# YiyanXu/DiFashion

Hardware: AMD Instinct MI355X
Metric: U-Net denoise steps/sec, 4-item outfit @ 64x64x4 latent (higher is better)
Workload: dtype bf16; 1 GPU; BASELINE configs[1]: one 4-item outfit, CFG on (4 branches) -> U-Net batch 16, DDIM-50 schedule, sd15 shape in_channels=8, 64x64x4 latents, 77 text tokens; one outfit per GPU; unet_batch=16, latent=64x64x4, parallelism=outfit-replicas x1 (no data-path collective)

## Files before the change

difashion_amd/csrc/winograd.hip:

```cpp
#include "gemm.h"

namespace {

DFH_DEVICE void load8(const bf16_t* p, float* f) { unpack8(*(const uint4*)p, f); }

__global__ __launch_bounds__(256) void wino_weight_kernel(const bf16_t* __restrict__ W, int ldw, bf16_t* __restrict__ U, int N, int C, int blocked) {
  const int n = blockIdx.x;
  const bf16_t* w = W + (long)n * ldw;
  for (int c = threadIdx.x; c < C; c += 256) {
    float g[3][3];
#pragma unroll
    for (int t = 0; t < 9; ++t) g[t / 3][t % 3] = bf2f(w[t * C + c]);
    float t4[4][3];
#pragma unroll
    for (int k = 0; k < 3; ++k) {
      t4[0][k] = g[0][k];
      t4[1][k] = 0.5f * (g[0][k] + g[1][k] + g[2][k]);
      t4[2][k] = 0.5f * (g[0][k] - g[1][k] + g[2][k]);
      t4[3][k] = g[2][k];
    }
#pragma unroll
    for (int i = 0; i < 4; ++i) {
      const float u[4] = {t4[i][0], 0.5f * (t4[i][0] + t4[i][1] + t4[i][2]), 0.5f * (t4[i][0] - t4[i][1] + t4[i][2]), t4[i][2]};
#pragma unroll
      for (int j = 0; j < 4; ++j) {
        const long off = blocked ? ((long)(n >> 4) * (C >> 6) + (c >> 6)) * 1024 + (n & 15) * 64 + (c & 63) : (long)n * C + c;
        U[(long)(i * 4 + j) * N * C + off] = f2bf(u[j]);
      }
    }
  }
}

__global__ __launch_bounds__(256) void wino_input_kernel(const bf16_t* __restrict__ g, bf16_t* __restrict__ V, int B, int H, int W, int C) {
  const int CH = C >> 3, TH = H >> 1, TW = W >> 1;
  const long Mt = (long)B * TH * TW;
  const long idx = (long)blockIdx.x * 256 + threadIdx.x;
  if (idx >= Mt * CH) return;
  const int ch = (int)(idx % CH);
  const long t = idx / CH;
  const int tx = (int)(t % TW), ty = (int)((t / TW) % TH), b = (int)(t / ((long)TW * TH));
  float d[4][4][8];
#pragma unroll
  for (int r = 0; r < 4; ++r) {
    const int y = 2 * ty - 1 + r;
#pragma unroll
    for (int s = 0; s < 4; ++s) {
      const int x = 2 * tx - 1 + s;
      if ((unsigned)y < (unsigned)H && (unsigned)x < (unsigned)W) load8(g + (((long)b * H + y) * W + x) * C + ch * 8, d[r][s]);
      else {
#pragma unroll
        for (int e = 0; e < 8; ++e) d[r][s][e] = 0.f;
      }
    }
  }
  float q[4][4][8];
#pragma unroll
  for (int s = 0; s < 4; ++s)
#pragma unroll
    for (int e = 0; e < 8; ++e) {
      q[0][s][e] = d[0][s][e] - d[2][s][e];
      q[1][s][e] = d[1][s][e] + d[2][s][e];
      q[2][s][e] = d[2][s][e] - d[1][s][e];
      q[3][s][e] = d[1][s][e] - d[3][s][e];
    }
#pragma unroll
  for (int i = 0; i < 4; ++i) {
    float v[4][8];
#pragma unroll
    for (int e = 0; e < 8; ++e) {
      v[0][e] = q[i][0][e] - q[i][2][e];
      v[1][e] = q[i][1][e] + q[i][2][e];
      v[2][e] = q[i][2][e] - q[i][1][e];
      v[3][e] = q[i][1][e] - q[i][3][e];
    }
#pragma unroll
    for (int j = 0; j < 4; ++j) *(uint4*)(V + ((long)(i * 4 + j) * Mt + t) * C + ch * 8) = pack8(v[j]);
  }
}

struct GnWinoArgs {
  const bf16_t* src0; const bf16_t* src1; int C0, C1;
  const float* gamma; const float* beta; float eps;
  bf16_t* V; int B, H, W, G;
  const bf16_t* Mprev; const float* pbias; const float* prowvec; int prv_ld, prv_off;
};

__global__ __launch_bounds__(256) void gn_wino_input_kernel(const GnWinoArgs a) {
  extern __shared__ __attribute__((aligned(16))) unsigned char smem[];
  const int g = blockIdx.x, b = blockIdx.y, tid = threadIdx.x;
  const int C = a.C0 + a.C1, cpg = C / a.G, upp = cpg >> 2, HW = a.H * a.W;
  const int cg = g * cpg, total = HW * upp;
  const int RS = cpg * 2 + 8;
  __shared__ float red[8];
  __shared__ __attribute__((aligned(16))) float gam_s[256], bet_s[256];
  if (tid < cpg) { gam_s[tid] = a.gamma[cg + tid]; bet_s[tid] = a.beta[cg + tid]; }
  float s = 0.f;
  if (a.Mprev) {
    const int TWp = a.W >> 1, tilesp = (a.H >> 1) * TWp;
    const long Mtp = (long)a.B * tilesp;
    for (int idx = tid; idx < tilesp * upp; idx += 256) {
      const int t = idx / upp, j = idx - t * upp, c = cg + j * 4;
      const int ty = t / TWp, tx = t - ty * TWp;
      float sm[2][4][4];
#pragma unroll
      for (int jj = 0; jj < 4; ++jj) {
        float m[4][4];
#pragma unroll
        for (int i = 0; i < 4; ++i) {
          const uint2 r = *(const uint2*)(a.Mprev + ((long)(i * 4 + jj) * Mtp + (long)b * tilesp + t) * a.C0 + c);
          m[i][0] = h16lo(r.x); m[i][1] = h16hi(r.x);
          m[i][2] = h16lo(r.y); m[i][3] = h16hi(r.y);
        }
#pragma unroll
        for (int e = 0; e < 4; ++e) {
          sm[0][jj][e] = m[0][e] + m[1][e] + m[2][e];
          sm[1][jj][e] = m[1][e] - m[2][e] - m[3][e];
        }
      }
      float4 add = *(const float4*)(a.pbias + c);
      if (a.prowvec) {
        const float4 rv = *(const float4*)(a.prowvec + (long)b * a.prv_ld + a.prv_off + c);
        add.x += rv.x; add.y += rv.y; add.z += rv.z; add.w += rv.w;
      }
      const float ad[4] = {add.x, add.y, add.z, add.w};
#pragma unroll
      for (int i = 0; i < 2; ++i)
#pragma unroll
        for (int jj = 0; jj < 2; ++jj) {
          float y[4];
#pragma unroll
          for (int e = 0; e < 4; ++e)
            y[e] = (jj == 0 ? sm[i][0][e] + sm[i][1][e] + sm[i][2][e] : sm[i][1][e] - sm[i][2][e] - sm[i][3][e]) + ad[e];
          uint2 r; r.x = pack2bf(y[0], y[1]); r.y = pack2bf(y[2], y[3]);
          const int p = (2 * ty + i) * a.W + 2 * tx + jj;
          *(uint2*)(smem + p * RS + j * 8) = r;
          s += (h16lo(r.x) + h16hi(r.x)) + (h16lo(r.y) + h16hi(r.y));
        }
    }
  } else
  for (int idx = tid; idx < total; idx += 256) {
    const int p = idx / upp, j = idx - p * upp, c = cg + j * 4;
    const uint2 r = c < a.C0 ? *(const uint2*)(a.src0 + ((long)b * HW + p) * a.C0 + c)
                             : *(const uint2*)(a.src1 + ((long)b * HW + p) * a.C1 + (c - a.C0));
    *(uint2*)(smem + p * RS + j * 8) = r;
    s += (h16lo(r.x) + h16hi(r.x)) + (h16lo(r.y) + h16hi(r.y));
  }
  s = wave_sum(s);
  if ((tid & 63) == 0) red[tid >> 6] = s;
  __syncthreads();
  const float n = (float)HW * (float)cpg;
  const float mean = ((red[0] + red[1]) + (red[2] + red[3])) / n;
  float q = 0.f;
  for (int idx = tid; idx < total; idx += 256) {
    const int p = idx / upp, j = idx - p * upp;
    const uint2 r = *(const uint2*)(smem + p * RS + j * 8);
    const float v[4] = {h16lo(r.x), h16hi(r.x), h16lo(r.y), h16hi(r.y)};
#pragma unroll
    for (int k = 0; k < 4; ++k) { const float d = v[k] - mean; q += d * d; }
  }
  q = wave_sum(q);
  if ((tid & 63) == 0) red[4 + (tid >> 6)] = q;
  __syncthreads();
  const float rstd = rsqrtf(((red[4] + red[5]) + (red[6] + red[7])) / n + a.eps);
  for (int idx = tid; idx < total; idx += 256) {
    const int p = idx / upp, j = idx - p * upp;
    uint2* slot = (uint2*)(smem + p * RS + j * 8);
    const uint2 r = *slot;
    const float4 gm = *(const float4*)(gam_s + j * 4), bt = *(const float4*)(bet_s + j * 4);
    const float y0 = silu_f((h16lo(r.x) - mean) * rstd * gm.x + bt.x);
    const float y1 = silu_f((h16hi(r.x) - mean) * rstd * gm.y + bt.y);
    const float y2 = silu_f((h16lo(r.y) - mean) * rstd * gm.z + bt.z);
    const float y3 = silu_f((h16hi(r.y) - mean) * rstd * gm.w + bt.w);
    uint2 o; o.x = pack2bf(y0, y1); o.y = pack2bf(y2, y3);
    *slot = o;
  }
  __syncthreads();
  const int TH = a.H >> 1, TW = a.W >> 1, tiles = TH * TW;
  const long Mt = (long)a.B * tiles;
  for (int idx = tid; idx < tiles * upp; idx += 256) {
    const int t = idx / upp, j = idx - t * upp;
    const int ty = t / TW, tx = t - ty * TW;
    float d[4][4][4];
#pragma unroll
    for (int r = 0; r < 4; ++r) {
      const int y = 2 * ty - 1 + r;
#pragma unroll
      for (int c4 = 0; c4 < 4; ++c4) {
        const int x = 2 * tx - 1 + c4;
        uint2 v = uint2{0u, 0u};
        if ((unsigned)y < (unsigned)a.H && (unsigned)x < (unsigned)a.W) v = *(const uint2*)(smem + (y * a.W + x) * RS + j * 8);
        d[r][c4][0] = h16lo(v.x); d[r][c4][1] = h16hi(v.x);
        d[r][c4][2] = h16lo(v.y); d[r][c4][3] = h16hi(v.y);
      }
    }
    float qv[4][4][4];
#pragma unroll
    for (int c4 = 0; c4 < 4; ++c4)
#pragma unroll
      for (int e = 0; e < 4; ++e) {
        qv[0][c4][e] = d[0][c4][e] - d[2][c4][e];
        qv[1][c4][e] = d[1][c4][e] + d[2][c4][e];
        qv[2][c4][e] = d[2][c4][e] - d[1][c4][e];
        qv[3][c4][e] = d[1][c4][e] - d[3][c4][e];
      }
    bf16_t* dst = a.V + ((long)b * tiles + t) * C + cg + j * 4;
#pragma unroll
    for (int i = 0; i < 4; ++i) {
      float v[4][4];
#pragma unroll
      for (int e = 0; e < 4; ++e) {
        v[0][e] = qv[i][0][e] - qv[i][2][e];
        v[1][e] = qv[i][1][e] + qv[i][2][e];
        v[2][e] = qv[i][2][e] - qv[i][1][e];
        v[3][e] = qv[i][1][e] - qv[i][3][e];
      }
#pragma unroll
      for (int jj = 0; jj < 4; ++jj) {
        uint2 o; o.x = pack2bf(v[jj][0], v[jj][1]); o.y = pack2bf(v[jj][2], v[jj][3]);
        *(uint2*)(dst + (long)(i * 4 + jj) * Mt * C) = o;
      }
    }
  }
}

__global__ __launch_bounds__(256) void wino_output_kernel(const bf16_t* __restrict__ Mb, bf16_t* __restrict__ out, const float* __restrict__ bias,
                                                          const float* __restrict__ rowvec, int rv_ld, int rv_off,
                                                          const bf16_t* __restrict__ resid, int B, int H, int W, int N) {
  const int CH = N >> 3, TH = H >> 1, TW = W >> 1;
  const long Mt = (long)B * TH * TW;
  const long idx = (long)blockIdx.x * 256 + threadIdx.x;
  if (idx >= Mt * CH) return;
  const int ch = (int)(idx % CH);
  const long t = idx / CH;
  const int tx = (int)(t % TW), ty = (int)((t / TW) % TH), b = (int)(t / ((long)TW * TH));
  float s[2][4][8];
#pragma unroll
  for (int j = 0; j < 4; ++j) {
    float m[4][8];
#pragma unroll
    for (int i = 0; i < 4; ++i) load8(Mb + ((long)(i * 4 + j) * Mt + t) * N + ch * 8, m[i]);
#pragma unroll
    for (int e = 0; e < 8; ++e) {
      s[0][j][e] = m[0][e] + m[1][e] + m[2][e];
      s[1][j][e] = m[1][e] - m[2][e] - m[3][e];
    }
  }
  float add[8];
  {
    const float4 b0 = *(const float4*)(bias + ch * 8), b1 = *(const float4*)(bias + ch * 8 + 4);
    add[0] = b0.x; add[1] = b0.y; add[2] = b0.z; add[3] = b0.w; add[4] = b1.x; add[5] = b1.y; add[6] = b1.z; add[7] = b1.w;
    if (rowvec) {
      const float* rv = rowvec + (long)b * rv_ld + rv_off + ch * 8;
      const float4 r0 = *(const float4*)rv, r1 = *(const float4*)(rv + 4);
      add[0] += r0.x; add[1] += r0.y; add[2] += r0.z; add[3] += r0.w; add[4] += r1.x; add[5] += r1.y; add[6] += r1.z; add[7] += r1.w;
    }
  }
#pragma unroll
  for (int i = 0; i < 2; ++i)
#pragma unroll
    for (int j = 0; j < 2; ++j) {
      float y[8];
#pragma unroll
      for (int e = 0; e < 8; ++e)
        y[e] = (j == 0 ? s[i][0][e] + s[i][1][e] + s[i][2][e] : s[i][1][e] - s[i][2][e] - s[i][3][e]) + add[e];
      const long pix = (((long)b * H + 2 * ty + i) * W + 2 * tx + j) * N + ch * 8;
      if (resid) {
        float r[8];
        load8(resid + pix, r);
#pragma unroll
        for (int e = 0; e < 8; ++e) y[e] += r[e];
      }
      *(uint4*)(out + pix) = pack8(y);
    }
}

}

namespace dfh {

int wino_weight_launch(const bf16_t* W, int ldw, bf16_t* U, int N, int C, int blocked, hipStream_t stream) {
  DFH_REQUIRE(W && U && N > 0 && C > 0 && ldw >= 9 * C, "bad argument");
  DFH_REQUIRE(!blocked || (N % 16 == 0 && C % 64 == 0), "blocked U needs N % 16 == 0 and C % 64 == 0");
  hipLaunchKernelGGL(wino_weight_kernel, dim3(N), dim3(256), 0, stream, W, ldw, U, N, C, blocked);
  return check_launch("wino_weight_kernel");
}

int wino_input_launch(const bf16_t* g, bf16_t* V, int B, int H, int W, int C, hipStream_t stream) {
  DFH_REQUIRE(g && V && B > 0 && H > 0 && W > 0 && (H & 1) == 0 && (W & 1) == 0 && C > 0 && C % 8 == 0, "even image sides, channels a multiple of 8");
  const long n = (long)B * (H / 2) * (W / 2) * (C / 8);
  ProfScope ps(PC_CONV3, 0.0, (double)B * H * W * C * 2.0 * 5.0, stream);
  hipLaunchKernelGGL(wino_input_kernel, dim3((unsigned)((n + 255) / 256)), dim3(256), 0, stream, g, V, B, H, W, C);
  return check_launch("wino_input_kernel");
}

bool gn_wino_ok(int C0, int C1, int G, int H, int W) {
  const int C = C0 + C1;
  if (G <= 0 || C % G) return false;
  const int cpg = C / G;
  return cpg % 4 == 0 && cpg <= 256 && C0 % 4 == 0 && (H & 1) == 0 && (W & 1) == 0 && (size_t)H * W * (cpg * 2 + 8) <= 96 * 1024;
}

int gn_wino_input_launch(const bf16_t* src0, int C0, const bf16_t* src1, int C1, const float* gamma, const float* beta, float eps, int G,
                         bf16_t* V, int B, int H, int W, hipStream_t stream, const bf16_t* Mprev, const float* pbias, const float* prowvec,
                         int prv_ld, int prv_off) {
  DFH_REQUIRE((src0 || Mprev) && gamma && beta && V && (C1 == 0 || src1), "null pointer");
  DFH_REQUIRE(!Mprev || (pbias && C1 == 0), "chained form: the previous conv's bias, one source");
  DFH_REQUIRE(gn_wino_ok(C0, C1, G, H, W), "shape not supported by the fused GroupNorm + input transform (gn_wino_ok)");
  GnWinoArgs a; a.src0 = src0; a.src1 = src1; a.C0 = C0; a.C1 = C1; a.gamma = gamma; a.beta = beta; a.eps = eps; a.V = V;
  a.B = B; a.H = H; a.W = W; a.G = G;
  a.Mprev = Mprev; a.pbias = pbias; a.prowvec = prowvec; a.prv_ld = prv_ld; a.prv_off = prv_off;
  const int C = C0 + C1;
  const size_t lds = (size_t)H * W * ((C / G) * 2 + 8);
  static size_t lds_set = 0;
  if (lds > 48 * 1024 && lds > lds_set) {
    (void)hipFuncSetAttribute((const void*)gn_wino_input_kernel, hipFuncAttributeMaxDynamicSharedMemorySize, 96 * 1024);
    lds_set = 96 * 1024;
  }
  ProfScope ps(PC_GNORM, 0.0, (double)B * H * W * C * 2.0 * 5.0, stream);
  hipLaunchKernelGGL(gn_wino_input_kernel, dim3(G, B), dim3(256), lds, stream, a);
  return check_launch("gn_wino_input_kernel");
}

int wino_output_launch(const bf16_t* Mb, bf16_t* out, const float* bias, const float* rowvec, int rv_ld, int rv_off, const bf16_t* resid,
                       int B, int H, int W, int N, hipStream_t stream) {
  DFH_REQUIRE(Mb && out && bias && B > 0 && H > 0 && W > 0 && (H & 1) == 0 && (W & 1) == 0 && N > 0 && N % 8 == 0, "even image sides, channels a multiple of 8");
  const long n = (long)B * (H / 2) * (W / 2) * (N / 8);
  ProfScope ps(PC_CONV3, 0.0, (double)B * H * W * N * 2.0 * (resid ? 6.0 : 5.0), stream);
  hipLaunchKernelGGL(wino_output_kernel, dim3((unsigned)((n + 255) / 256)), dim3(256), 0, stream, Mb, out, bias, rowvec, rv_ld, rv_off, resid,
                     B, H, W, N);
  return check_launch("wino_output_kernel");
}

}
```

Baseline: 65.43 steps/s.

## Restructure fused GroupNorm+Winograd input kernel with register-resident slabs and templated vector width

Rewrites the fused GroupNorm + Winograd input-transform kernel as a template over vector width, units per thread and the chained form. Each thread now keeps its pixel slab in registers and applies the normalization from those registers instead of re-reading LDS. The statistics loops are unrolled four at a time, the output transform is split per row pair to cut register pressure, and block IDs are swizzled across XCDs. It also uses 512-thread blocks with launch bounds for higher occupancy, at the cost of more template instantiations and extra register use that could spill.

Result: no change. 65.68 steps/s (median of 6 runs) (+0.4%).

```diff
diff --git a/difashion_amd/csrc/winograd.hip b/difashion_amd/csrc/winograd.hip
--- a/difashion_amd/csrc/winograd.hip
+++ b/difashion_amd/csrc/winograd.hip
@@ -85,65 +85,154 @@
   const bf16_t* Mprev; const float* pbias; const float* prowvec; int prv_ld, prv_off;
 };
 
-__global__ __launch_bounds__(256) void gn_wino_input_kernel(const GnWinoArgs a) {
+template <int VEC> struct GwUnit { uint32_t w[VEC / 2]; };
+template <int VEC> DFH_DEVICE GwUnit<VEC> gw_zero() {
+  GwUnit<VEC> r;
+#pragma unroll
+  for (int k = 0; k < VEC / 2; ++k) r.w[k] = 0u;
+  return r;
+}
+template <int VEC> DFH_DEVICE GwUnit<VEC> gw_load(const void* p) {
+  GwUnit<VEC> r;
+  if constexpr (VEC == 8) { const uint4 v = *(const uint4*)p; r.w[0] = v.x; r.w[1] = v.y; r.w[2] = v.z; r.w[3] = v.w; }
+  else { const uint2 v = *(const uint2*)p; r.w[0] = v.x; r.w[1] = v.y; }
+  return r;
+}
+template <int VEC> DFH_DEVICE void gw_store(void* p, const GwUnit<VEC>& r) {
+  if constexpr (VEC == 8) *(uint4*)p = uint4{r.w[0], r.w[1], r.w[2], r.w[3]};
+  else *(uint2*)p = uint2{r.w[0], r.w[1]};
+}
+template <int VEC> DFH_DEVICE void gw_unpack(const GwUnit<VEC>& r, float* f) {
+#pragma unroll
+  for (int k = 0; k < VEC / 2; ++k) { f[2 * k] = h16lo(r.w[k]); f[2 * k + 1] = h16hi(r.w[k]); }
+}
+template <int VEC> DFH_DEVICE GwUnit<VEC> gw_pack(const float* f) {
+  GwUnit<VEC> r;
+#pragma unroll
+  for (int k = 0; k < VEC / 2; ++k) r.w[k] = pack2bf(f[2 * k], f[2 * k + 1]);
+  return r;
+}
+template <int VEC, int UNITS, bool CHAIN>
+__global__ __launch_bounds__(512, UNITS <= 8 ? 4 : 2) void gn_wino_input_kernel(const GnWinoArgs a, const int ppb) {
   extern __shared__ __attribute__((aligned(16))) unsigned char smem[];
-  const int g = blockIdx.x, b = blockIdx.y, tid = threadIdx.x;
-  const int C = a.C0 + a.C1, cpg = C / a.G, upp = cpg >> 2, HW = a.H * a.W;
-  const int cg = g * cpg, total = HW * upp;
-  const int RS = cpg * 2 + 8;
-  __shared__ float red[8];
-  __shared__ __attribute__((aligned(16))) float gam_s[256], bet_s[256];
-  if (tid < cpg) { gam_s[tid] = a.gamma[cg + tid]; bet_s[tid] = a.beta[cg + tid]; }
+  __shared__ float red[32];
+  const int tid = threadIdx.x;
+  int id = blockIdx.x;
+  {
+    const int per = gridDim.x >> 3;
+    if (id < per * 8) id = (id & 7) * per + (id >> 3);
+  }
+  const int b = id / a.G, g = id - b * a.G;
+  const int C = a.C0 + a.C1, cpg = C / a.G, upp = cpg / VEC, HW = a.H * a.W;
+  const int RS = cpg * 2 + (VEC == 8 ? 16 : 8);
+  const int pp = tid / upp, j = tid - pp * upp;
+  const bool active = pp < ppb;
+  const int c = g * cpg + j * VEC;
+  const int TH = a.H >> 1, TW = a.W >> 1, tiles = TH * TW;
+  const long Mt = (long)a.B * tiles;
+  auto unit_pixel = [&](int u, bool* ok) -> int {
+    if constexpr (CHAIN) {
+      const int t = pp + (u >> 2) * ppb;
+      *ok = active && t < tiles;
+      const int ty = t / TW, tx = t - ty * TW;
+      return (2 * ty + ((u >> 1) & 1)) * a.W + 2 * tx + (u & 1);
+    } else {
+      const int p = pp + u * ppb;
+      *ok = active && p < HW;
+      return p;
+    }
+  };
+  GwUnit<VEC> v[UNITS];
+  if constexpr (CHAIN) {
+    float add[VEC];
+#pragma unroll
+    for (int e = 0; e < VEC; e += 4) {
+      float4 x = *(const float4*)(a.pbias + c + e);
+      if (a.prowvec) {
+        const float4 rv = *(const float4*)(a.prowvec + (long)b * a.prv_ld + a.prv_off + c + e);
+        x.x += rv.x; x.y += rv.y; x.z += rv.z; x.w += rv.w;
+      }
+      add[e] = x.x; add[e + 1] = x.y; add[e + 2] = x.z; add[e + 3] = x.w;
+    }
+#pragma unroll
+    for (int k = 0; k < UNITS / 4; ++k) {
+      const int t = pp + k * ppb;
+#pragma unroll
+      for (int u = 0; u < 4; ++u) v[k * 4 + u] = gw_zero<VEC>();
+      if (active && t < tiles) {
+        const bf16_t* mp = a.Mprev + ((long)b * tiles + t) * a.C0 + c;
+        float y[2][2][VEC];
+#pragma unroll
+        for (int jj = 0; jj < 4; ++jj) {
+          float m[4][VEC];
+#pragma unroll
+          for (int i = 0; i < 4; ++i) gw_unpack<VEC>(gw_load<VEC>(mp + (long)(i * 4 + jj) * Mt * a.C0), m[i]);
+#pragma unroll
+          for (int e = 0; e < VEC; ++e) {
+            const float s0 = m[0][e] + m[1][e] + m[2][e], s1 = m[1][e] - m[2][e] - m[3][e];
+            if (jj == 0) { y[0][0][e] = s0; y[1][0][e] = s1; }
+            if (jj == 1) { y[0][0][e] += s0; y[1][0][e] += s1; y[0][1][e] = s0; y[1][1][e] = s1; }
+            if (jj == 2) { y[0][0][e] += s0; y[1][0][e] += s1; y[0][1][e] -= s0; y[1][1][e] -= s1; }
+            if (jj == 3) { y[0][1][e] -= s0; y[1][1][e] -= s1; }
+          }
+        }
+#pragma unroll
+        for (int i = 0; i < 2; ++i)
+#pragma unroll
+          for (int jj = 0; jj < 2; ++jj) {
+#pragma unroll
+            for (int e = 0; e < VEC; ++e) y[i][jj][e] += add[e];
+            v[k * 4 + i * 2 + jj] = gw_pack<VEC>(y[i][jj]);
+          }
+      }
+    }
+  } else {
+    const bool first = c < a.C0;
+    const bf16_t* src = first ? a.src0 + (long)b * HW * a.C0 + c : a.src1 + (long)b * HW * a.C1 + (c - a.C0);
+    const int ldc = first ? a.C0 : a.C1;
+#pragma unroll
+    for (int u = 0; u < UNITS; ++u) {
+      const int p = pp + u * ppb;
+      v[u] = gw_zero<VEC>();
+      if (active && p < HW) v[u] = gw_load<VEC>(src + (long)p * ldc);
+    }
+  }
+#pragma unroll
+  for (int u = 0; u < UNITS; ++u) {
+    bool ok;
+    const int p = unit_pixel(u, &ok);
+    if (ok) gw_store<VEC>(smem + p * RS + j * (VEC * 2), v[u]);
+  }
+  __syncthreads();
+  const int upp4 = cpg >> 2, total = HW * upp4;
+  const int sdp = 256 / upp4, sdj = 256 - sdp * upp4, sp0 = tid / upp4, sj0 = tid - sp0 * upp4;
   float s = 0.f;
-  if (a.Mprev) {
-    const int TWp = a.W >> 1, tilesp = (a.H >> 1) * TWp;
-    const long Mtp = (long)a.B * tilesp;
-    for (int idx = tid; idx < tilesp * upp; idx += 256) {
-      const int t = idx / upp, j = idx - t * upp, c = cg + j * 4;
-      const int ty = t / TWp, tx = t - ty * TWp;
-      float sm[2][4][4];
-#pragma unroll
-      for (int jj = 0; jj < 4; ++jj) {
-        float m[4][4];
-#pragma unroll
-        for (int i = 0; i < 4; ++i) {
-          const uint2 r = *(const uint2*)(a.Mprev + ((long)(i * 4 + jj) * Mtp + (long)b * tilesp + t) * a.C0 + c);
-          m[i][0] = h16lo(r.x); m[i][1] = h16hi(r.x);
-          m[i][2] = h16lo(r.y); m[i][3] = h16hi(r.y);
+  if (tid < 256) {
+    const int lim = CHAIN ? tiles * upp4 : total;
+    for (int idx = tid, p = sp0, jq = sj0; idx < lim; idx += 1024) {
+      constexpr int NP = CHAIN ? 4 : 1;
+      uint2 r[4][NP];
+#pragma unroll
+      for (int k = 0; k < 4; ++k) {
+        if (idx + 256 * k < lim) {
+          if constexpr (CHAIN) {
+            const int ty = p / TW, tx = p - ty * TW;
+#pragma unroll
+            for (int e = 0; e < 4; ++e) r[k][e] = *(const uint2*)(smem + ((2 * ty + (e >> 1)) * a.W + 2 * tx + (e & 1)) * RS + jq * 8);
+          } else {
+            r[k][0] = *(const uint2*)(smem + p * RS + jq * 8);
+          }
         }
-#pragma unroll
-        for (int e = 0; e < 4; ++e) {
-          sm[0][jj][e] = m[0][e] + m[1][e] + m[2][e];
-          sm[1][jj][e] = m[1][e] - m[2][e] - m[3][e];
+        p += sdp; jq += sdj;
+        if (jq >= upp4) { jq -= upp4; ++p; }
+      }
+#pragma unroll
+      for (int k = 0; k < 4; ++k)
+        if (idx + 256 * k < lim) {
+#pragma unroll
+          for (int e = 0; e < NP; ++e) s += (h16lo(r[k][e].x) + h16hi(r[k][e].x)) + (h16lo(r[k][e].y) + h16hi(r[k][e].y));
         }
-      }
-      float4 add = *(const float4*)(a.pbias + c);
-      if (a.prowvec) {
-        const float4 rv = *(const float4*)(a.prowvec + (long)b * a.prv_ld + a.prv_off + c);
-        add.x += rv.x; add.y += rv.y; add.z += rv.z; add.w += rv.w;
-      }
-      const float ad[4] = {add.x, add.y, add.z, add.w};
-#pragma unroll
-      for (int i = 0; i < 2; ++i)
-#pragma unroll
-        for (int jj = 0; jj < 2; ++jj) {
-          float y[4];
-#pragma unroll
-          for (int e = 0; e < 4; ++e)
-            y[e] = (jj == 0 ? sm[i][0][e] + sm[i][1][e] + sm[i][2][e] : sm[i][1][e] - sm[i][2][e] - sm[i][3][e]) + ad[e];
-          uint2 r; r.x = pack2bf(y[0], y[1]); r.y = pack2bf(y[2], y[3]);
-          const int p = (2 * ty + i) * a.W + 2 * tx + jj;
-          *(uint2*)(smem + p * RS + j * 8) = r;
-          s += (h16lo(r.x) + h16hi(r.x)) + (h16lo(r.y) + h16hi(r.y));
-        }
-    }
-  } else
-  for (int idx = tid; idx < total; idx += 256) {
-    const int p = idx / upp, j = idx - p * upp, c = cg + j * 4;
-    const uint2 r = c < a.C0 ? *(const uint2*)(a.src0 + ((long)b * HW + p) * a.C0 + c)
-                             : *(const uint2*)(a.src1 + ((long)b * HW + p) * a.C1 + (c - a.C0));
-    *(uint2*)(smem + p * RS + j * 8) = r;
-    s += (h16lo(r.x) + h16hi(r.x)) + (h16lo(r.y) + h16hi(r.y));
+    }
   }
   s = wave_sum(s);
   if ((tid & 63) == 0) red[tid >> 6] = s;
@@ -151,74 +240,79 @@
   const float n = (float)HW * (float)cpg;
   const float mean = ((red[0] + red[1]) + (red[2] + red[3])) / n;
   float q = 0.f;
-  for (int idx = tid; idx < total; idx += 256) {
-    const int p = idx / upp, j = idx - p * upp;
-    const uint2 r = *(const uint2*)(smem + p * RS + j * 8);
-    const float v[4] = {h16lo(r.x), h16hi(r.x), h16lo(r.y), h16hi(r.y)};
-#pragma unroll
-    for (int k = 0; k < 4; ++k) { const float d = v[k] - mean; q += d * d; }
+  if (tid < 256) {
+    for (int idx = tid, p = sp0, jq = sj0; idx < total; idx += 1024) {
+      uint2 r[4];
+#pragma unroll
+      for (int k = 0; k < 4; ++k) {
+        if (idx + 256 * k < total) r[k] = *(const uint2*)(smem + p * RS + jq * 8);
+        p += sdp; jq += sdj;
+        if (jq >= upp4) { jq -= upp4; ++p; }
+      }
+#pragma unroll
+      for (int k = 0; k < 4; ++k)
+        if (idx + 256 * k < total) {
+          const float f[4] = {h16lo(r[k].x), h16hi(r[k].x), h16lo(r[k].y), h16hi(r[k].y)};
+#pragma unroll
+          for (int e = 0; e < 4; ++e) { const float d = f[e] - mean; q += d * d; }
+        }
+    }
   }
   q = wave_sum(q);
-  if ((tid & 63) == 0) red[4 + (tid >> 6)] = q;
+  if ((tid & 63) == 0) red[16 + (tid >> 6)] = q;
   __syncthreads();
-  const float rstd = rsqrtf(((red[4] + red[5]) + (red[6] + red[7])) / n + a.eps);
-  for (int idx = tid; idx < total; idx += 256) {
-    const int p = idx / upp, j = idx - p * upp;
-    uint2* slot = (uint2*)(smem + p * RS + j * 8);
-    const uint2 r = *slot;
-    const float4 gm = *(const float4*)(gam_s + j * 4), bt = *(const float4*)(bet_s + j * 4);
-    const float y0 = silu_f((h16lo(r.x) - mean) * rstd * gm.x + bt.x);
-    const float y1 = silu_f((h16hi(r.x) - mean) * rstd * gm.y + bt.y);
-    const float y2 = silu_f((h16lo(r.y) - mean) * rstd * gm.z + bt.z);
-    const float y3 = silu_f((h16hi(r.y) - mean) * rstd * gm.w + bt.w);
-    uint2 o; o.x = pack2bf(y0, y1); o.y = pack2bf(y2, y3);
-    *slot = o;
+  const float rstd = rsqrtf(((red[16] + red[17]) + (red[18] + red[19])) / n + a.eps);
+  if (active) {
+    float gm[VEC], bt[VEC];
+#pragma unroll
+    for (int e = 0; e < VEC; e += 4) {
+      const float4 x = *(const float4*)(a.gamma + c + e), y = *(const float4*)(a.beta + c + e);
+      gm[e] = x.x; gm[e + 1] = x.y; gm[e + 2] = x.z; gm[e + 3] = x.w;
+      bt[e] = y.x; bt[e + 1] = y.y; bt[e + 2] = y.z; bt[e + 3] = y.w;
+    }
+#pragma unroll
+    for (int u = 0; u < UNITS; ++u) {
+      bool ok;
+      const int p = unit_pixel(u, &ok);
+      if (ok) {
+        float f[VEC];
+        gw_unpack<VEC>(v[u], f);
+#pragma unroll
+        for (int k = 0; k < VEC; ++k) f[k] = silu_f((f[k] - mean) * rstd * gm[k] + bt[k]);
+        gw_store<VEC>(smem + p * RS + j * (VEC * 2), gw_pack<VEC>(f));
+      }
+    }
   }
   __syncthreads();
-  const int TH = a.H >> 1, TW = a.W >> 1, tiles = TH * TW;
-  const long Mt = (long)a.B * tiles;
-  for (int idx = tid; idx < tiles * upp; idx += 256) {
-    const int t = idx / upp, j = idx - t * upp;
+  if (!active) return;
+  for (int it = pp; it < 4 * tiles; it += ppb) {
+    const int t = it >> 2, i = it & 3;
     const int ty = t / TW, tx = t - ty * TW;
-    float d[4][4][4];
-#pragma unroll
-    for (int r = 0; r < 4; ++r) {
-      const int y = 2 * ty - 1 + r;
-#pragma unroll
-      for (int c4 = 0; c4 < 4; ++c4) {
-        const int x = 2 * tx - 1 + c4;
-        uint2 v = uint2{0u, 0u};
-        if ((unsigned)y < (unsigned)a.H && (unsigned)x < (unsigned)a.W) v = *(const uint2*)(smem + (y * a.W + x) * RS + j * 8);
-        d[r][c4][0] = h16lo(v.x); d[r][c4][1] = h16hi(v.x);
-        d[r][c4][2] = h16lo(v.y); d[r][c4][3] = h16hi(v.y);
-      }
-    }
-    float qv[4][4][4];
-#pragma unroll
-    for (int c4 = 0; c4 < 4; ++c4)
-#pragma unroll
-      for (int e = 0; e < 4; ++e) {
-        qv[0][c4][e] = d[0][c4][e] - d[2][c4][e];
-        qv[1][c4][e] = d[1][c4][e] + d[2][c4][e];
-        qv[2][c4][e] = d[2][c4][e] - d[1][c4][e];
-        qv[3][c4][e] = d[1][c4][e] - d[3][c4][e];
-      }
-    bf16_t* dst = a.V + ((long)b * tiles + t) * C + cg + j * 4;
-#pragma unroll
-    for (int i = 0; i < 4; ++i) {
-      float v[4][4];
-#pragma unroll
-      for (int e = 0; e < 4; ++e) {
-        v[0][e] = qv[i][0][e] - qv[i][2][e];
-        v[1][e] = qv[i][1][e] + qv[i][2][e];
-        v[2][e] = qv[i][2][e] - qv[i][1][e];
-        v[3][e] = qv[i][1][e] - qv[i][3][e];
-      }
-#pragma unroll
-      for (int jj = 0; jj < 4; ++jj) {
-        uint2 o; o.x = pack2bf(v[jj][0], v[jj][1]); o.y = pack2bf(v[jj][2], v[jj][3]);
-        *(uint2*)(dst + (long)(i * 4 + jj) * Mt * C) = o;
-      }
+    const int ra = i == 0 ? 0 : i == 2 ? 2 : 1, rb = i == 0 ? 2 : i == 2 ? 1 : i == 1 ? 2 : 3;
+    const int ya = 2 * ty - 1 + ra, yb = 2 * ty - 1 + rb;
+    float qv[4][VEC];
+#pragma unroll
+    for (int c4 = 0; c4 < 4; ++c4) {
+      const int x = 2 * tx - 1 + c4;
+      GwUnit<VEC> da = gw_zero<VEC>(), db = gw_zero<VEC>();
+      if ((unsigned)x < (unsigned)a.W) {
+        if ((unsigned)ya < (unsigned)a.H) da = gw_load<VEC>(smem + (ya * a.W + x) * RS + j * (VEC * 2));
+        if ((unsigned)yb < (unsigned)a.H) db = gw_load<VEC>(smem + (yb * a.W + x) * RS + j * (VEC * 2));
+      }
+      float fa[VEC], fb[VEC];
+      gw_unpack<VEC>(da, fa);
+      gw_unpack<VEC>(db, fb);
+#pragma unroll
+      for (int e = 0; e < VEC; ++e) qv[c4][e] = i == 1 ? fa[e] + fb[e] : fa[e] - fb[e];
+    }
+    bf16_t* dst = a.V + ((long)(i * 4) * Mt + (long)b * tiles + t) * C + c;
+#pragma unroll
+    for (int jj = 0; jj < 4; ++jj) {
+      const int ca = jj == 0 ? 0 : jj == 2 ? 2 : 1, cb = jj == 0 ? 2 : jj == 2 ? 1 : jj == 1 ? 2 : 3;
+      float o[VEC];
+#pragma unroll
+      for (int e = 0; e < VEC; ++e) o[e] = jj == 1 ? qv[ca][e] + qv[cb][e] : qv[ca][e] - qv[cb][e];
+      gw_store<VEC>(dst + (long)jj * Mt * C, gw_pack<VEC>(o));
     }
   }
 }
@@ -300,25 +394,45 @@
   return cpg % 4 == 0 && cpg <= 256 && C0 % 4 == 0 && (H & 1) == 0 && (W & 1) == 0 && (size_t)H * W * (cpg * 2 + 8) <= 96 * 1024;
 }
 
+template <int VEC, int UNITS, bool CHAIN>
+static int gn_wino_input_dispatch(const GnWinoArgs& a, int blocks, int threads, int ppb, size_t lds, hipStream_t stream) {
+  static bool lds_set = false;
+  if (lds > 48 * 1024 && !lds_set) {
+    (void)hipFuncSetAttribute((const void*)gn_wino_input_kernel<VEC, UNITS, CHAIN>, hipFuncAttributeMaxDynamicSharedMemorySize, 96 * 1024);
+    lds_set = true;
+  }
+  hipLaunchKernelGGL((gn_wino_input_kernel<VEC, UNITS, CHAIN>), dim3(blocks), dim3(threads), lds, stream, a, ppb);
+  return check_launch("gn_wino_input_kernel");
+}
+
 int gn_wino_input_launch(const bf16_t* src0, int C0, const bf16_t* src1, int C1, const float* gamma, const float* beta, float eps, int G,
                          bf16_t* V, int B, int H, int W, hipStream_t stream, const bf16_t* Mprev, const float* pbias, const float* prowvec,
                          int prv_ld, int prv_off) {
   DFH_REQUIRE((src0 || Mprev) && gamma && beta && V && (C1 == 0 || src1), "null pointer");
   DFH_REQUIRE(!Mprev || (pbias && C1 == 0), "chained form: the previous conv's bias, one source");
+  DFH_REQUIRE(B > 0 && (long)B * G < (1L << 30), "bad batch");
   DFH_REQUIRE(gn_wino_ok(C0, C1, G, H, W), "shape not supported by the fused GroupNorm + input transform (gn_wino_ok)");
   GnWinoArgs a; a.src0 = src0; a.src1 = src1; a.C0 = C0; a.C1 = C1; a.gamma = gamma; a.beta = beta; a.eps = eps; a.V = V;
   a.B = B; a.H = H; a.W = W; a.G = G;
   a.Mprev = Mprev; a.pbias = pbias; a.prowvec = prowvec; a.prv_ld = prv_ld; a.prv_off = prv_off;
-  const int C = C0 + C1;
-  const size_t lds = (size_t)H * W * ((C / G) * 2 + 8);
-  static size_t lds_set = 0;
-  if (lds > 48 * 1024 && lds > lds_set) {
-    (void)hipFuncSetAttribute((const void*)gn_wino_input_kernel, hipFuncAttributeMaxDynamicSharedMemorySize, 96 * 1024);
-    lds_set = 96 * 1024;
-  }
+  const int C = C0 + C1, cpg = C / G, HW = H * W;
+  const bool v8 = !Mprev && cpg % 8 == 0 && C0 % 8 == 0 && (size_t)HW * (cpg * 2 + 16) <= 96 * 1024;
+  const int upp = cpg / (v8 ? 8 : 4);
+  const size_t lds = (size_t)HW * (cpg * 2 + (v8 ? 16 : 8));
+  const int threads = (long)(Mprev ? HW / 4 : HW) * upp <= 256 ? 256 : 512;
+  const int ppb = threads / upp;
+  const int units = Mprev ? 4 * ((HW / 4 + ppb - 1) / ppb) : (HW + ppb - 1) / ppb;
+  DFH_REQUIRE(ppb >= 1 && units <= (v8 ? 16 : 32), "slab too large for the register-resident statistics");
   ProfScope ps(PC_GNORM, 0.0, (double)B * H * W * C * 2.0 * 5.0, stream);
-  hipLaunchKernelGGL(gn_wino_input_kernel, dim3(G, B), dim3(256), lds, stream, a);
-  return check_launch("gn_wino_input_kernel");
+  const int blocks = G * B;
+  if (Mprev)
+    return units <= 8 ? gn_wino_input_dispatch<4, 8, true>(a, blocks, threads, ppb, lds, stream)
+                      : gn_wino_input_dispatch<4, 32, true>(a, blocks, threads, ppb, lds, stream);
+  if (v8) return units <= 4   ? gn_wino_input_dispatch<8, 4, false>(a, blocks, threads, ppb, lds, stream)
+                 : units <= 8 ? gn_wino_input_dispatch<8, 8, false>(a, blocks, threads, ppb, lds, stream)
+                              : gn_wino_input_dispatch<8, 16, false>(a, blocks, threads, ppb, lds, stream);
+  return units <= 8 ? gn_wino_input_dispatch<4, 8, false>(a, blocks, threads, ppb, lds, stream)
+                    : gn_wino_input_dispatch<4, 32, false>(a, blocks, threads, ppb, lds, stream);
 }
 
 int wino_output_launch(const bf16_t* Mb, bf16_t* out, const float* bias, const float* rowvec, int rv_ld, int rv_off, const bf16_t* resid,
```
